# XPU-Forces/mojo_opset

Measured on AMD Instinct MI355X. Metric: MojoPagedDecodeGQA tokens/s (Llama-3-8B shape, bf16, 1/8 MI355X), higher is better.
Workload: dtype bf16; 1 GPU; MojoPagedDecodeGQA bf16, B=64, 32q/8kv, head_dim=128, page=16, ctx=4096 uniform, AABB, random block tables (BASELINE configs[1]); per_gpu_batch=64, parallelism=replicas x1 (no collective on this path)

## Files before the change

### mojo_opset_amd/csrc/paged_decode_common.h

```cpp
#pragma once

namespace mojo {

struct DecodePair {
  int b[2] = {0, -1};
  int len[2] = {0, 0};
  int chunk[2] = {DEC_TILE, DEC_TILE};
  int n_first = 8;
};
__device__ __forceinline__ int decode_pick(const int (&v)[2], int u) { return u ? v[1] : v[0]; }

__device__ __forceinline__ DecodePair decode_pair(const DecodeArgs& a, int lane, int p) {
  DecodePair pr;
  const int cap = a.n_chunks * a.chunk_tokens;
  int len = -1;
  if (lane < a.batch) len = a.max_pages > 0 ? max(min(a.seq_lens[lane], cap), 0) : 0;
  int rank = lane;
  if (__ballot(lane < a.batch && len != __builtin_amdgcn_readfirstlane(len)) != 0) {
    rank = 0;
    for (int o = 0; o < a.batch; ++o) {
      const int lo = __builtin_amdgcn_readlane(len, o);
      rank += (lo > len || (lo == len && o < lane)) ? 1 : 0;
    }
  }
  const unsigned long long first = __ballot(lane < a.batch && rank == p);
  const unsigned long long second = __ballot(lane < a.batch && rank == a.batch - 1 - p && a.batch - 1 - p > p);
  pr.b[0] = __builtin_ctzll(first);
  pr.len[0] = __builtin_amdgcn_readlane(len, pr.b[0]);
  if (second) {
    pr.b[1] = __builtin_ctzll(second);
    pr.len[1] = __builtin_amdgcn_readlane(len, pr.b[1]);
  }
  const int sum = pr.len[0] + pr.len[1];
  pr.n_first = pr.len[1] <= 0 ? 8 : min(max((8 * pr.len[0] + sum / 2) / sum, 1), 7);
#pragma unroll
  for (int u = 0; u < 2; ++u) {
    const int n_u = u ? 8 - pr.n_first : pr.n_first;
    int c = n_u > 0 ? (pr.len[u] + n_u - 1) / n_u : DEC_TILE;
    c = max(c, 128);
    pr.chunk[u] = ((c + DEC_TILE - 1) / DEC_TILE) * DEC_TILE;
  }
  return pr;
}

struct DecodeRow {
  int b = 0, chunk = 0;
  int seq_len = 0, chunk_tokens = 0;
  int tok_begin = 0, tok_end = 0;
  bool has_work = false;

  __device__ __forceinline__ void cut() {
    tok_begin = chunk * chunk_tokens;
    has_work = seq_len > 0 && tok_begin < seq_len;
    tok_end = has_work ? min(seq_len, tok_begin + chunk_tokens) : tok_begin + 1;
  }
  __device__ __forceinline__ int n_chunks_seq() const { return (seq_len + chunk_tokens - 1) / chunk_tokens; }
};

template <bool SWA>
__device__ __forceinline__ int decode_row_len(const DecodeArgs& a, int b, DecodeWin& win) {
  if constexpr (SWA) return a.max_pages > 0 ? decode_swa_row(a, b, win) : 0;
  else return a.max_pages > 0 ? decode_seq_len(a, b) : 0;
}
__device__ __forceinline__ DecodeRow decode_row(const DecodeArgs& a, int b, int chunk, int seq_len) {
  DecodeRow r;
  r.b = b;
  r.chunk = chunk;
  r.seq_len = seq_len;
  r.chunk_tokens = decode_seq_chunk(a, seq_len);
  r.cut();
  return r;
}

__device__ __forceinline__ DecodeRow decode_row(const DecodePair& pr, int wave_id) {
  DecodeRow r;
  const int u = wave_id < pr.n_first ? 0 : 1;
  r.b = decode_pick(pr.b, u);
  r.chunk = u ? wave_id - pr.n_first : wave_id;
  r.seq_len = r.b >= 0 ? decode_pick(pr.len, u) : 0;
  r.chunk_tokens = decode_pick(pr.chunk, u);
  if (r.b < 0) r.b = pr.b[0];
  r.cut();
  return r;
}

struct DecodeHoles {
  static constexpr int SCAN = 4;
  int p1, first_neg = 0x7fffffff;
  int v[SCAN];

  __device__ __forceinline__ DecodeHoles(const DecodeArgs& a, int tok_end) : p1((tok_end + a.page - 1) / a.page) {
    if (p1 > a.max_pages) { first_neg = a.max_pages; p1 = a.max_pages; }
  }
  __device__ __forceinline__ void issue(const int32_t* table, int lane, int base) {
#pragma unroll
    for (int u = 0; u < SCAN; ++u) v[u] = table[min(base + u * 64 + lane, p1 - 1)];
  }
  __device__ __forceinline__ void reduce(int lane, int base) {
#pragma unroll
    for (int u = 0; u < SCAN; ++u) {
      const unsigned long long neg = __ballot(v[u] < 0 && base + u * 64 + lane < p1);
      if (neg && first_neg == 0x7fffffff) first_neg = base + u * 64 + __builtin_ctzll(neg);
    }
  }
  __device__ __forceinline__ void finish(const int32_t* table, int lane) {
    reduce(lane, 0);
    for (int base = 64 * SCAN; base < p1 && first_neg == 0x7fffffff; base += 64 * SCAN) {
      issue(table, lane, base);
      reduce(lane, base);
    }
  }
};

template <typename T>
struct Store16 {
  void* out;
  __device__ __forceinline__ void operator()(int64_t at, f32x4 x) const {
    typename vec_of<T, 4>::type o;
#pragma unroll
    for (int e = 0; e < 4; ++e) o[e] = static_cast<T>(x[e]);
    *reinterpret_cast<typename vec_of<T, 4>::type*>(static_cast<T*>(out) + at) = o;
  }
};

template <bool PAIRED, bool GROUPED, typename Store>
__device__ __forceinline__ void decode_lds_merge(const DecodeArgs& a, const float* s_part, int D, int G, int kvh,
                                                 const DecodeRow& row, const DecodePair& pr, Store store) {
  static_assert(!(PAIRED && GROUPED), "the paired form is never grouped");
  const int stride = D + 2;
  __syncthreads();
  const int per_head = D / 4;
  constexpr int UNITS = PAIRED ? 2 : 1;
  for (int item = threadIdx.x; item < UNITS * G * per_head; item += blockDim.x) {
    const int u = item / (G * per_head);
    const int rest = item - u * (G * per_head);
    const int g = rest / per_head, d0 = (rest - g * per_head) * 4;
    int ub, ulen, uchunk, slot0, uwaves;
    if constexpr (PAIRED) {
      ub = decode_pick(pr.b, u); ulen = decode_pick(pr.len, u); uchunk = decode_pick(pr.chunk, u);
      slot0 = u ? pr.n_first : 0;
      uwaves = u ? 8 - pr.n_first : pr.n_first;
      if (ub < 0) continue;
    } else {
      ub = row.b; ulen = row.seq_len; uchunk = row.chunk_tokens; slot0 = 0; uwaves = static_cast<int>(blockDim.x >> 6);
    }
    int n_chunks_seq = ulen <= 0 ? 0 : min((ulen + uchunk - 1) / uchunk, uwaves);
    bool partial = false;
    if constexpr (GROUPED) {
      if (a.fuse_group > 0) {
        const int total = ulen <= 0 ? 0 : (ulen + uchunk - 1) / uchunk;
        partial = total > uwaves;
        n_chunks_seq = min(max(total - static_cast<int>(blockIdx.x) * uwaves, 0), uwaves);
        if (blockIdx.x > 0 && n_chunks_seq == 0) continue;
      }
    }
    if (n_chunks_seq == 0 && a.leave_empty) continue;
    const int h = decode_head(a, kvh, g, G);
    float mx = -INFINITY;
    for (int c = 0; c < n_chunks_seq; ++c) mx = fmaxf(mx, s_part[((slot0 + c) * G + g) * stride + D]);
    f32x4 num = {0.f, 0.f, 0.f, 0.f};
    float den = 0.f;
    for (int c = 0; c < n_chunks_seq; ++c) {
      const float* src = s_part + ((slot0 + c) * G + g) * stride;
      const float w = exp2f(src[D] - mx);
      den = fmaf(w, src[D + 1], den);
      num += f32x4{src[d0], src[d0 + 1], src[d0 + 2], src[d0 + 3]} * w;
    }
    if (partial) {
      const int64_t slot = (static_cast<int64_t>(blockIdx.y) * a.n_chunks + blockIdx.x) * G + g;
      *reinterpret_cast<f32x4*>(a.ws_acc + slot * D + d0) = num;
      if (d0 == 0) { a.ws_ml[slot * 2 + 0] = mx; a.ws_ml[slot * 2 + 1] = den; }
      continue;
    }
    const float inv = n_chunks_seq > 0 ? 1.0f / den : 0.f;
    store((static_cast<int64_t>(ub) * a.hq + h) * D + d0, num * inv);
  }
}

template <int ND, typename Store>
__device__ __forceinline__ void decode_split_finish(const DecodeArgs& a, int G, int kvh, const DecodeRow& row, int tl, int g4,
                                                    const f32x4 (&o)[ND], float m, float l, Store store) {
  constexpr int D = ND * 16;
  if (tl >= G) return;
  if (row.n_chunks_seq() == 1) {
    const int h = decode_head(a, kvh, tl, G);
    const float inv = 1.0f / l;
    const int64_t at = (static_cast<int64_t>(row.b) * a.hq + h) * D + 4 * g4;
#pragma unroll
    for (int dt = 0; dt < ND; ++dt) store(at + dt * 16, o[dt] * inv);
    return;
  }
  const int64_t slot = (static_cast<int64_t>(blockIdx.y) * a.n_chunks + row.chunk) * G + tl;
  float* dst = a.ws_acc + slot * D + 4 * g4;
#pragma unroll
  for (int dt = 0; dt < ND; ++dt) *reinterpret_cast<f32x4*>(dst + dt * 16) = o[dt];
  if (g4 == 0) {
    a.ws_ml[slot * 2 + 0] = m;
    a.ws_ml[slot * 2 + 1] = l;
  }
}

template <typename MM, int NS, int ND>
__device__ __forceinline__ void decode_softmax_step(const float (&x)[NS][4], float& m, float& l, f32x4 (&o)[ND],
                                                    typename MM::frag4 (&pf)[NS]) {
  float mx = fmaxf(fmaxf(x[0][0], x[0][1]), fmaxf(x[0][2], x[0][3]));
#pragma unroll
  for (int ss = 1; ss < NS; ++ss) mx = fmaxf(mx, fmaxf(fmaxf(x[ss][0], x[ss][1]), fmaxf(x[ss][2], x[ss][3])));
  mx = xor_max_16_32(mx);
  float ref = m;
  if (mx - m > 8.0f) ref = mx;
  if (!__all(ref == m)) {
    const float alpha = m == ref ? 1.f : fast_exp2(m - ref);
    l *= alpha;
#pragma unroll
    for (int dt = 0; dt < ND; ++dt) o[dt] *= alpha;
    m = ref;
  }
  const float ms = m == -INFINITY ? 0.f : m;
#pragma unroll
  for (int ss = 0; ss < NS; ++ss) {
    float p[4];
#pragma unroll
    for (int i = 0; i < 4; ++i) p[i] = fast_exp2(x[ss][i] - ms);
    l += (p[0] + p[1]) + (p[2] + p[3]);
    pf[ss] = MM::pack(p[0], p[1], p[2], p[3]);
  }
}

}
```

### mojo_opset_amd/csrc/paged_decode_mfma.h

```cpp
#pragma once

namespace mojo {

template <typename T> struct dec_mma;
template <> struct dec_mma<bf16_t> {
  typedef bf16x8 frag8;
  typedef s16x4 frag4;
  static __device__ __forceinline__ f32x4 qk(frag8 a, frag8 b, f32x4 c) { return __builtin_amdgcn_mfma_f32_16x16x32_bf16(a, b, c, 0, 0, 0); }
  static __device__ __forceinline__ f32x4 pv(frag4 a, frag4 b, f32x4 c) { return __builtin_amdgcn_mfma_f32_16x16x16bf16_1k(a, b, c, 0, 0, 0); }
  static __device__ __forceinline__ frag4 pack(float p0, float p1, float p2, float p3) {
    const bf16x4 v = {static_cast<bf16_t>(p0), static_cast<bf16_t>(p1), static_cast<bf16_t>(p2), static_cast<bf16_t>(p3)};
    return __builtin_bit_cast(frag4, v);
  }
  static __device__ __forceinline__ frag4 from_lds(s16x4 v) { return v; }
};
template <> struct dec_mma<f16_t> {
  typedef f16x8 frag8;
  typedef f16x4 frag4;
  static __device__ __forceinline__ f32x4 qk(frag8 a, frag8 b, f32x4 c) { return __builtin_amdgcn_mfma_f32_16x16x32_f16(a, b, c, 0, 0, 0); }
  static __device__ __forceinline__ f32x4 pv(frag4 a, frag4 b, f32x4 c) { return __builtin_amdgcn_mfma_f32_16x16x16f16(a, b, c, 0, 0, 0); }
  static __device__ __forceinline__ frag4 pack(float p0, float p1, float p2, float p3) {
    const f16x4 v = {static_cast<f16_t>(p0), static_cast<f16_t>(p1), static_cast<f16_t>(p2), static_cast<f16_t>(p3)};
    return v;
  }
  static __device__ __forceinline__ frag4 from_lds(s16x4 v) { return __builtin_bit_cast(f16x4, v); }
};

constexpr int DECM_TILE = 16;

template <typename T, int DK , bool NT, int MODE, bool SWA = false >
__global__ __launch_bounds__(MODE != DEC_SPLIT ? 512 : 64) void decode_mfma_kernel(DecodeArgs a, int G) {
  constexpr bool FUSED = MODE != DEC_SPLIT;
  constexpr bool PAIRED = MODE == DEC_PAIRED;
  static_assert(!(SWA && PAIRED), "the paired form takes no window");
  constexpr int D = DK * 32, ND = D / 16;
  constexpr int ROWB = D * 2;
  constexpr int NP = D / 16;
  constexpr int RPB = 8 / NP;
  constexpr int NS = DK == 2 ? 2 : 1;
  constexpr int STEP = DECM_TILE * NS;
  typedef typename pack8<T>::vec V8;
  typedef dec_mma<T> MM;
  const int lane = threadIdx.x & 63;
  const int tl = lane & 15, g4 = lane >> 4;
  const int wave_id = FUSED ? __builtin_amdgcn_readfirstlane(static_cast<int>(threadIdx.x >> 6)) : 0;
  const int chunk0 = FUSED ? static_cast<int>(blockIdx.x) * static_cast<int>(blockDim.x >> 6) + wave_id : static_cast<int>(blockIdx.x);
  const int b0 = blockIdx.y / a.hkv;
  const int kvh = blockIdx.y % a.hkv;

  DecodeWin win;
  DecodePair pr;
  DecodeRow row;
  if constexpr (PAIRED) { pr = decode_pair(a, lane, b0); row = decode_row(pr, wave_id); }
  else row = decode_row(a, b0, chunk0, decode_row_len<SWA>(a, b0, win));
  const int b = row.b, tok_begin = row.tok_begin, tok_end = row.tok_end;
  const bool has_work = row.has_work;
  if (!FUSED && !has_work) return;

  const int hq_l = min(tl, G - 1);
  constexpr int NL = D / 64;
  typename MM::frag8 qf[NL][2];

  f32x4 o[ND];
#pragma unroll
  for (int dt = 0; dt < ND; ++dt) o[dt] = f32x4{0.f, 0.f, 0.f, 0.f};
  float m = -INFINITY, l = 0.f;

  const int32_t* table = a.tables + static_cast<int64_t>(b) * a.table_stride;
  DecodeHoles holes(a, tok_end);

  constexpr int CPR = D / 8;
  constexpr int RPI = 64 / CPR;
  constexpr int NV = 16 / RPI;
  const int kt8 = lane & 7, kc8 = lane >> 3;
  const int vr = lane / CPR, vc = lane % CPR;
  const T* kbase = static_cast<const T*>(a.kc) + (kvh >> a.hshift) * a.c_head + kc8 * 8;
  const T* vbase = static_cast<const T*>(a.vc) + (kvh >> a.hshift) * a.c_head + vc * 8;
  const int last_tile = ((tok_end - 1) / DECM_TILE) * DECM_TILE;
  const int last_page = a.max_pages - 1;

  constexpr int IDW = 60;
  static_assert(IDW % (3 * NS) == 0 && IDW + 2 * NS <= 64, "windows change between rounds; a round's requests stay inside one");
  auto id_window = [&](int s_base) -> int {
    int tu = min(tok_begin + DECM_TILE * (s_base + lane), last_tile);
    if constexpr (SWA) tu = decode_swa_real(win, tu);
    return table[min(tu >> a.page_shift, last_page)];
  };
  {
    const int h = decode_head(a, kvh, hq_l, G);
    const T* qp = static_cast<const T*>(a.q) + (static_cast<int64_t>(b) * a.hq + h) * a.dim;
#pragma unroll
    for (int L = 0; L < NL; ++L)
#pragma unroll
      for (int p = 0; p < 2; ++p) qf[L][p] = *reinterpret_cast<const typename MM::frag8*>(qp + (8 * L + 2 * g4 + p) * 8);
  }
  int idw = 0, idn = 0, id_base = 0;
  if (has_work) {
    idw = id_window(0);
    idn = id_window(IDW);
    if constexpr (!SWA) holes.issue(table, lane, 0);
  }
  struct Tile { V8 k[NS][2][NL]; V8 v[NS][NV]; int lp[NS]; };
  auto ld = [&](const T* p) -> V8 {
    if constexpr (NT) return __builtin_nontemporal_load(reinterpret_cast<const V8*>(p));
    else return *reinterpret_cast<const V8*>(p);
  };
  auto load_tile = [&](Tile& t, int t0) {
    const int s0 = __builtin_amdgcn_readfirstlane((t0 - tok_begin) / DECM_TILE) - id_base;
#pragma unroll
    for (int ss = 0; ss < NS; ++ss) {
      int tu = min(t0 + DECM_TILE * ss, last_tile);
      if constexpr (SWA) tu = decode_swa_real(win, tu);
      const int lp = tu >> a.page_shift;
      t.lp[ss] = lp;
      const int phys = max(__builtin_amdgcn_readlane(idw, s0 + ss), 0);
      const int64_t pg = static_cast<int64_t>(phys) * a.c_blk + static_cast<int64_t>(tu - (lp << a.page_shift)) * a.c_tok;
#pragma unroll
      for (int j = 0; j < 2; ++j)
#pragma unroll
        for (int L = 0; L < NL; ++L) t.k[ss][j][L] = ld(kbase + pg + static_cast<int64_t>(8 * j + kt8) * a.c_tok + L * 64);
#pragma unroll
      for (int u = 0; u < NV; ++u) t.v[ss][u] = ld(vbase + pg + static_cast<int64_t>(RPI * u + vr) * a.c_tok);
    }
  };

  extern __shared__ float s_part[];
  const int n_waves = FUSED ? static_cast<int>(blockDim.x >> 6) : 1;
  char* const v_img = reinterpret_cast<char*>(s_part + (FUSED ? n_waves * G * (D + 2) : 0)) + wave_id * (NS * 16 * ROWB);
  const unsigned v_u32 = static_cast<unsigned>(reinterpret_cast<size_t>(v_img));
  unsigned w_off[NV];
#pragma unroll
  for (int u = 0; u < NV; ++u) {
    const int row = RPI * u + vr;
    const int fw = (row / RPB) & (NP - 1);
    w_off[u] = row * ROWB + (((vc >> 1) ^ fw) << 5) + (vc & 1) * 16;
  }
  const int rrow = 4 * g4 + (tl >> 2);
  const int fr = (rrow / RPB) & (NP - 1);
  const unsigned r_base = v_u32 + rrow * ROWB + (tl & 3) * 8;

  auto process = [&](Tile& t, int t0) {
#pragma unroll
    for (int ss = 0; ss < NS; ++ss)
      if (t.lp[ss] >= holes.first_neg) {
        V8 z = {};
#pragma unroll
        for (int j = 0; j < 2; ++j)
#pragma unroll
          for (int L = 0; L < NL; ++L) t.k[ss][j][L] = z;
#pragma unroll
        for (int u = 0; u < NV; ++u) t.v[ss][u] = z;
      }
    const bool full = t0 + STEP <= tok_end;
    int rt[NS];
    bool edge[NS], any_edge = false;
#pragma unroll
    for (int ss = 0; ss < NS; ++ss) {
      rt[ss] = t0 + DECM_TILE * ss;
      edge[ss] = false;
      if constexpr (SWA) {
        rt[ss] = decode_swa_real(win, rt[ss]);
        edge[ss] = decode_swa_edge(win, rt[ss]);
        any_edge = any_edge || edge[ss];
      }
    }
    float x[NS][4];
#pragma unroll
    for (int ss = 0; ss < NS; ++ss) {
      f32x4 c[2][2];
#pragma unroll
      for (int j = 0; j < 2; ++j)
#pragma unroll
        for (int p = 0; p < 2; ++p) {
          c[j][p] = f32x4{0.f, 0.f, 0.f, 0.f};
#pragma unroll
          for (int L = 0; L < NL; ++L) c[j][p] = MM::qk(__builtin_bit_cast(typename MM::frag8, t.k[ss][j][L]), qf[L][p], c[j][p]);
        }
#pragma unroll
      for (int u = 0; u < NV; ++u) {
        const bool vrow_ok = full || (t0 + DECM_TILE * ss + RPI * u + vr) < tok_end;
        V8 z = {};
        *reinterpret_cast<V8*>(v_img + ss * (16 * ROWB) + w_off[u]) = vrow_ok ? t.v[ss][u] : z;
      }
#pragma unroll
      for (int i = 0; i < 4; ++i) {
        const float xa = c[0][1][i], ya = c[1][0][i];
        const auto sw = __builtin_amdgcn_permlane32_swap(__builtin_bit_cast(unsigned, xa), __builtin_bit_cast(unsigned, ya), false, false);
        const float own = lane < 32 ? c[0][0][i] : c[1][1][i];
        const float oth = __builtin_bit_cast(float, lane < 32 ? sw[1] : sw[0]);
        x[ss][i] = (own + oth) * a.scale_log2;
      }
    }
    if (!full || any_edge) {
#pragma unroll
      for (int ss = 0; ss < NS; ++ss)
#pragma unroll
        for (int i = 0; i < 4; ++i) {
          bool ok = t0 + DECM_TILE * ss + 4 * g4 + i < tok_end;
          if constexpr (SWA) ok = ok && (!edge[ss] || decode_swa_vis(win, rt[ss] + 4 * g4 + i));
          if (!ok) x[ss][i] = -INFINITY;
        }
    }
    typename MM::frag4 pf[NS];
    decode_softmax_step<MM>(x, m, l, o, pf);
#pragma unroll
    for (int dt = 0; dt < ND; ++dt)
#pragma unroll
      for (int ss = 0; ss < NS; ++ss) {
        const s16x4 vt = __builtin_amdgcn_ds_read_tr16_b64_v4i16(
            reinterpret_cast<__attribute__((address_space(3))) s16x4*>(static_cast<uintptr_t>(r_base + ss * (16 * ROWB) + ((dt ^ fr) << 5))));
        o[dt] = MM::pv(MM::from_lds(vt), pf[ss], o[dt]);
      }
  };

  Tile ta, tb, tc;
  if (has_work) {
    auto scan_rest = [&]() { if constexpr (!SWA) holes.finish(table, lane); };
    int t0 = tok_begin;
    load_tile(ta, tok_begin);
    if (tok_begin + 4 * STEP < tok_end) {
      load_tile(tb, tok_begin + STEP);
      scan_rest();
      for (;;) {
        const int t_win = tok_begin + DECM_TILE * (id_base + IDW);
        do {
          load_tile(tc, t0 + 2 * STEP);
          process(ta, t0);
          load_tile(ta, t0 + 3 * STEP);
          process(tb, t0 + STEP);
          load_tile(tb, t0 + 4 * STEP);
          process(tc, t0 + 2 * STEP);
          t0 += 3 * STEP;
        } while (t0 + 4 * STEP < tok_end && t0 < t_win);
        if (t0 < t_win) break;
        asm volatile("v_mov_b32 %0, %1" : "=v"(idw) : "v"(idn));
        id_base += IDW;
        idn = id_window(id_base + IDW);
        if (t0 + 4 * STEP >= tok_end) break;
      }
    } else {
      if (tok_begin + STEP < tok_end) load_tile(tb, tok_begin + STEP);
      scan_rest();
    }
    if (t0 + 2 * STEP < tok_end) load_tile(tc, t0 + 2 * STEP);
    process(ta, t0);
    if (t0 + STEP < tok_end) {
      if (t0 + 3 * STEP < tok_end) load_tile(ta, t0 + 3 * STEP);
      process(tb, t0 + STEP);
      if (t0 + 2 * STEP < tok_end) {
        process(tc, t0 + 2 * STEP);
        if (t0 + 3 * STEP < tok_end) process(ta, t0 + 3 * STEP);
      }
    }
  }

  l = xor_sum_16_32(l);
  if constexpr (FUSED) {
    if (tl < G) {
      float* dst = s_part + (wave_id * G + tl) * (D + 2);
#pragma unroll
      for (int dt = 0; dt < ND; ++dt) *reinterpret_cast<f32x4*>(dst + dt * 16 + 4 * g4) = o[dt];
      if (g4 == 0) { dst[D] = m; dst[D + 1] = l; }
    }
    decode_lds_merge<PAIRED, !PAIRED>(a, s_part, D, G, kvh, row, pr, Store16<T>{a.out});
    return;
  }
  decode_split_finish(a, G, kvh, row, tl, g4, o, m, l, Store16<T>{a.out});
}

}
```

Before: 396,300 tokens/s.

## Batch block-table hole scan loads and restructure decode tail pipeline

Issues up to eight groups of block-table hole-scan loads up front, before the first KV tiles, so their latency overlaps the tile loads instead of running as serial load-then-ballot rounds. The tail processing is rewritten around a single remaining-token count, and the second tile is now loaded unconditionally. It also adds an amdgpu_waves_per_eu(2) hint to the kernel. The extra scan registers and the occupancy hint may raise register pressure or cause spills, and the unconditional second tile load reads a clamped tile even for short chunks.

```diff
diff --git a/mojo_opset_amd/csrc/paged_decode_common.h b/mojo_opset_amd/csrc/paged_decode_common.h
--- a/mojo_opset_amd/csrc/paged_decode_common.h
+++ b/mojo_opset_amd/csrc/paged_decode_common.h
@@ -92,20 +92,25 @@
   __device__ __forceinline__ DecodeHoles(const DecodeArgs& a, int tok_end) : p1((tok_end + a.page - 1) / a.page) {
     if (p1 > a.max_pages) { first_neg = a.max_pages; p1 = a.max_pages; }
   }
-  __device__ __forceinline__ void issue(const int32_t* table, int lane, int base) {
-#pragma unroll
-    for (int u = 0; u < SCAN; ++u) v[u] = table[min(base + u * 64 + lane, p1 - 1)];
-  }
-  __device__ __forceinline__ void reduce(int lane, int base) {
+  __device__ __forceinline__ void issue(const int32_t* table, int lane, int base) { issue(v, table, lane, base); }
+  __device__ __forceinline__ void reduce(int lane, int base) { reduce(v, lane, base); }
+  __device__ __forceinline__ void issue(int (&w)[SCAN], const int32_t* table, int lane, int base) const {
+#pragma unroll
+    for (int u = 0; u < SCAN; ++u) w[u] = table[min(base + u * 64 + lane, p1 - 1)];
+  }
+  __device__ __forceinline__ void reduce(const int (&w)[SCAN], int lane, int base) {
 #pragma unroll
     for (int u = 0; u < SCAN; ++u) {
-      const unsigned long long neg = __ballot(v[u] < 0 && base + u * 64 + lane < p1);
+      const unsigned long long neg = __ballot(w[u] < 0 && base + u * 64 + lane < p1);
       if (neg && first_neg == 0x7fffffff) first_neg = base + u * 64 + __builtin_ctzll(neg);
     }
   }
   __device__ __forceinline__ void finish(const int32_t* table, int lane) {
     reduce(lane, 0);
-    for (int base = 64 * SCAN; base < p1 && first_neg == 0x7fffffff; base += 64 * SCAN) {
+    rest(table, lane, 64 * SCAN);
+  }
+  __device__ __forceinline__ void rest(const int32_t* table, int lane, int base) {
+    for (; base < p1 && first_neg == 0x7fffffff; base += 64 * SCAN) {
       issue(table, lane, base);
       reduce(lane, base);
     }
diff --git a/mojo_opset_amd/csrc/paged_decode_mfma.h b/mojo_opset_amd/csrc/paged_decode_mfma.h
--- a/mojo_opset_amd/csrc/paged_decode_mfma.h
+++ b/mojo_opset_amd/csrc/paged_decode_mfma.h
@@ -29,7 +29,7 @@
 constexpr int DECM_TILE = 16;
 
 template <typename T, int DK , bool NT, int MODE, bool SWA = false >
-__global__ __launch_bounds__(MODE != DEC_SPLIT ? 512 : 64) void decode_mfma_kernel(DecodeArgs a, int G) {
+__global__ __launch_bounds__(MODE != DEC_SPLIT ? 512 : 64) __attribute__((amdgpu_waves_per_eu(2))) void decode_mfma_kernel(DecodeArgs a, int G) {
   constexpr bool FUSED = MODE != DEC_SPLIT;
   constexpr bool PAIRED = MODE == DEC_PAIRED;
   static_assert(!(SWA && PAIRED), "the paired form takes no window");
@@ -95,10 +95,18 @@
       for (int p = 0; p < 2; ++p) qf[L][p] = *reinterpret_cast<const typename MM::frag8*>(qp + (8 * L + 2 * g4 + p) * 8);
   }
   int idw = 0, idn = 0, id_base = 0;
+  constexpr int SCAN_PAGES = 64 * DecodeHoles::SCAN, SCAN_MORE = 7;
+  int scan_more[SCAN_MORE][DecodeHoles::SCAN];
   if (has_work) {
     idw = id_window(0);
     idn = id_window(IDW);
-    if constexpr (!SWA) holes.issue(table, lane, 0);
+    if constexpr (!SWA) {
+      holes.issue(table, lane, 0);
+      if (holes.p1 > SCAN_PAGES) {
+#pragma unroll
+        for (int e = 0; e < SCAN_MORE; ++e) holes.issue(scan_more[e], table, lane, SCAN_PAGES * (e + 1));
+      }
+    }
   }
   struct Tile { V8 k[NS][2][NL]; V8 v[NS][NV]; int lp[NS]; };
   auto ld = [&](const T* p) -> V8 {
@@ -215,12 +223,18 @@
 
   Tile ta, tb, tc;
   if (has_work) {
-    auto scan_rest = [&]() { if constexpr (!SWA) holes.finish(table, lane); };
     int t0 = tok_begin;
     load_tile(ta, tok_begin);
+    load_tile(tb, tok_begin + STEP);
+    if constexpr (!SWA) {
+      holes.reduce(lane, 0);
+      if (holes.p1 > SCAN_PAGES) {
+#pragma unroll
+        for (int e = 0; e < SCAN_MORE; ++e) holes.reduce(scan_more[e], lane, SCAN_PAGES * (e + 1));
+        holes.rest(table, lane, SCAN_PAGES * (SCAN_MORE + 1));
+      }
+    }
     if (tok_begin + 4 * STEP < tok_end) {
-      load_tile(tb, tok_begin + STEP);
-      scan_rest();
       for (;;) {
         const int t_win = tok_begin + DECM_TILE * (id_base + IDW);
         do {
@@ -238,20 +252,28 @@
         idn = id_window(id_base + IDW);
         if (t0 + 4 * STEP >= tok_end) break;
       }
+    }
+    const int left = tok_end - t0;
+    if (left > 2 * STEP) {
+      load_tile(tc, t0 + 2 * STEP);
+      process(ta, t0);
+      if (left > 3 * STEP) {
+        load_tile(ta, t0 + 3 * STEP);
+        process(tb, t0 + STEP);
+        process(tc, t0 + 2 * STEP);
+        process(ta, t0 + 3 * STEP);
+      } else {
+        process(tb, t0 + STEP);
+        process(tc, t0 + 2 * STEP);
+      }
     } else {
-      if (tok_begin + STEP < tok_end) load_tile(tb, tok_begin + STEP);
-      scan_rest();
-    }
-    if (t0 + 2 * STEP < tok_end) load_tile(tc, t0 + 2 * STEP);
-    process(ta, t0);
-    if (t0 + STEP < tok_end) {
-      if (t0 + 3 * STEP < tok_end) load_tile(ta, t0 + 3 * STEP);
-      process(tb, t0 + STEP);
-      if (t0 + 2 * STEP < tok_end) {
-        process(tc, t0 + 2 * STEP);
-        if (t0 + 3 * STEP < tok_end) process(ta, t0 + 3 * STEP);
-      }
-    }
+      process(ta, t0);
+      if (left > STEP) {
+        asm volatile("");
+        process(tb, t0 + STEP);
+      }
+    }
+    asm volatile("" : : "v"(idn));
   }
 
   l = xor_sum_16_32(l);
```

After: 395,100 tokens/s. Within noise of the previous version (-0.3%).
